# youtalk/opencv-ar

Hardware: AMD Instinct MI355X
Metric: frames/sec at 1920x1080, 16 markers/frame; 1/2/4/8 MI355X (higher is better)
Workload: dtype u8

## Files before the change

opencv-ar_amd/csrc/api.hip:

```cpp
#include "kernels.h"
#include "lanes_core.h"
#include <algorithm>
#include <cstdio>
#include <cstdlib>
#include <cstring>
#include <mutex>
#include <new>
#include <string>
#include <thread>
#include <vector>

using namespace ocvar;

static_assert(sizeof(TemplateRec) == sizeof(OcvarTemplate) && sizeof(TemplateRec) == 48, "CvarTemplate layout");
static_assert(MAX_SIZE_CLASSES == OCVAR_MAX_TEMPLATE_SIZES, "size classes");
static_assert(sizeof(CameraRec) == sizeof(OcvarCamera) && sizeof(CameraRec) == 248, "CvarCamera layout");
static_assert(sizeof(MarkerRec) == sizeof(OcvarMarker) && sizeof(MarkerRec) == 184, "CvarMarker layout");
static_assert(sizeof(BoardEntry) == sizeof(OcvarBoardMarker) && sizeof(BoardEntry) == 72, "OcvarBoardMarker layout");
static_assert(sizeof(BoardPose) == sizeof(OcvarBoardPose) && sizeof(BoardPose) == 192, "OcvarBoardPose layout");

struct OcvarGate {
    int device = 0;
    std::mutex mu;
    LaneSched sched;
// ... 1055 lines not shown
    for (int i = 0; i < n && i < max_quads; i++)
        for (int k = 0; k < 8; k++) quads[8 * i + k] = (int)sq[8 * (size_t)i + k];
    return OCVAR_OK;
}

extern "C" int ocvar_hip_debug_gray(OcvarHip* c, int frame, uint8_t* h) {
    if (!c || !h || frame < 0 || frame >= c->ws.n_frames) return OCVAR_E_ARG;
    HIP_TRY(c, hipSetDevice(c->device));
    const int W = c->ws.W, H = c->ws.H, pitch = gray_pitch(W);
    const size_t plane = (size_t)gray_plane_bytes(W, H);
    std::vector<uint8_t> g(plane);
    HIP_TRY(c, hipMemcpy(g.data(), c->ws.gray + frame * plane, plane, hipMemcpyDeviceToHost));
    for (int y = 0; y < H; y++)
        for (int x = 0; x < W; x++) h[(size_t)y * W + x] = g[(size_t)y * pitch + gray_col(x)];
    return OCVAR_OK;
}

extern "C" int ocvar_hip_debug_binary(OcvarHip* c, int frame, uint8_t* h) {
    if (!c || !h || frame < 0 || frame >= c->ws.n_frames) return OCVAR_E_ARG;
    HIP_TRY(c, hipSetDevice(c->device));
    const int sw = c->ws.sw, sh = c->ws.sh, ns = c->ws.ns;
    const size_t bytes = (size_t)nbr_plane_bytes(ns, sh);
    std::vector<uint8_t> nbr(bytes);
    HIP_TRY(c, hipMemcpy(nbr.data(), c->ws.nbr_frame + (size_t)frame * bytes, bytes, hipMemcpyDeviceToHost));
    for (int y = 0; y < sh; y++)
        for (int x = 0; x < sw; x++) h[(size_t)y * sw + x] = nbr_bit(nbr.data(), x, y, ns) ? 255 : 0;
    return OCVAR_OK;
}

extern "C" int ocvar_hip_debug_masks(OcvarHip* c, int frame, uint8_t* h) {
    if (!c || !h || frame < 0 || frame >= c->ws.n_frames) return OCVAR_E_ARG;
    HIP_TRY(c, hipSetDevice(c->device));
    const int sw = c->ws.sw, sh = c->ws.sh, ns = c->ws.ns;
    const size_t bytes = (size_t)nbr_plane_bytes(ns, sh);
    std::vector<uint8_t> nbr(bytes);
    HIP_TRY(c, hipMemcpy(nbr.data(), c->ws.nbr_frame + (size_t)frame * bytes, bytes, hipMemcpyDeviceToHost));
    for (int y = 0; y < sh; y++)
        for (int x = 0; x < sw; x++) h[(size_t)y * sw + x] = (uint8_t)nbr_of(nbr.data(), x, y, ns);
    return OCVAR_OK;
}

extern "C" int ocvar_hip_debug_frame_quads(OcvarHip* c, int frame, int* quads, int* n_quads) {
    if (!c || !quads || !n_quads || frame < 0 || frame >= c->ws.n_frames) return OCVAR_E_ARG;
    HIP_TRY(c, hipSetDevice(c->device));
    int n = 0;
    HIP_TRY(c, hipMemcpy(&n, c->ws.n_squares + frame, sizeof(int), hipMemcpyDeviceToHost));
    const int lim = c->ws.maxq < OCVAR_MAX_QUADS ? c->ws.maxq : OCVAR_MAX_QUADS;
    std::vector<float> sq((size_t)lim * 8);
    HIP_TRY(c, hipMemcpy(sq.data(), c->ws.squares + (size_t)frame * c->ws.maxq * 8, sq.size() * sizeof(float), hipMemcpyDeviceToHost));
    *n_quads = n;
    for (int i = 0; i < n && i < lim; i++)
        for (int k = 0; k < 8; k++) quads[8 * i + k] = (int)sq[8 * (size_t)i + k];
    return OCVAR_OK;
}

extern "C" int ocvar_hip_debug_candidates(OcvarHip* c, int frame, OcvarCandidate* cands, int max_cands, int* n_cands) {
    if (!c || !cands || !n_cands || frame < 0 || frame >= c->ws.n_frames) return OCVAR_E_ARG;
    HIP_TRY(c, hipSetDevice(c->device));
    int nsq = 0;
    HIP_TRY(c, hipMemcpy(&nsq, c->ws.n_squares + frame, sizeof(int), hipMemcpyDeviceToHost));
    if (nsq > c->ws.maxq) nsq = c->ws.maxq;
    const Workspace& w = c->ws;
    const Library& L = c->lib;
    const size_t first = (size_t)frame * w.maxq;
    std::vector<SquareRec> recs(nsq > 0 ? nsq : 1);
    std::vector<long long> codes((size_t)(nsq > 0 ? nsq : 1) * w.n_sizes);
    std::vector<int> match((size_t)(nsq > 0 ? nsq : 1) * w.max_match);
    if (nsq > 0) {
        HIP_TRY(c, hipMemcpy(recs.data(), w.sq_recs + first, nsq * sizeof(SquareRec), hipMemcpyDeviceToHost));
        HIP_TRY(c, hipMemcpy(codes.data(), w.sq_codes + first * w.n_sizes, codes.size() * sizeof(long long), hipMemcpyDeviceToHost));
        HIP_TRY(c, hipMemcpy(match.data(), w.sq_match + first * w.max_match, match.size() * sizeof(int), hipMemcpyDeviceToHost));
    }
    std::vector<int> orient_of(L.n_groups(), 0);
    long long n = 0;
    for (int i = 0; i < nsq; i++) {
        const SquareRec& r = recs[i];
        if (r.n_match < 0) continue;
        if (n >= max_cands) {
            n += w.n_templates;
            continue;
        }
        const int* m = match.data() + (size_t)i * w.max_match;
        for (int k = 0; k < r.n_match; k++) orient_of[match_group(m[k])] = match_orient_of(m[k]);
        int sh = 0;
        for (int j = 0; j < w.n_templates; j++, n++) {
            const int orient = orient_of[L.group_of[j]];
            sh = (sh + orient_shift(orient)) & 3;
            if (n >= max_cands) continue;
            OcvarCandidate& o = cands[n];
            o.markerId = i;
            o.templateId = j;
            o.orient = orient;
            o.valid = 1;
            o.bit = codes[(size_t)i * w.n_sizes + L.size_of[j]];
            shift_square(r.square, sh, o.square);
            std::memcpy(o.patPoint, r.patPoint, sizeof o.patPoint);
        }
        for (int k = 0; k < r.n_match; k++) orient_of[match_group(m[k])] = 0;
    }
    *n_cands = n > 0x7fffffff ? 0x7fffffff : (int)n;
    return OCVAR_OK;
}

extern "C" int ocvar_hip_stage_ms(OcvarHip* c, float* ms, int n) {
    if (!c || !ms || n < 1 || c->pending) return OCVAR_E_ARG;
    int k = 0;
    for (; k < 11 && k < n; k++)
        if (hipEventElapsedTime(&ms[k], c->ev[k], c->ev[k + 1]) != hipSuccess) ms[k] = -1.f;
    if (k < n && k == 11) {
        if (hipEventElapsedTime(&ms[11], c->ev[0], c->ev[12]) != hipSuccess) ms[11] = -1.f;
        k = 12;
    }
    return k;
}

extern "C" int ocvar_hip_stage_stamps(OcvarHip* c, void* ref_event, float* ms, int n) {
    if (!c || !ref_event || !ms || n < 1 || c->pending) return OCVAR_E_ARG;
    int k = 0;
    for (; k < 13 && k < n; k++)
        if (hipEventElapsedTime(&ms[k], (hipEvent_t)ref_event, c->ev[k]) != hipSuccess) {
            (void)hipGetLastError();
            ms[k] = -1.f;
        }
    return k;
}

__global__ void calib_copy_dword_kernel(const unsigned* src, unsigned* dst, size_t n) {
    for (size_t i = (size_t)blockIdx.x * blockDim.x + threadIdx.x; i < n; i += (size_t)gridDim.x * blockDim.x) dst[i] = src[i] + 1u;
}

extern "C" int ocvar_hip_debug_calibrate(OcvarHip* c, size_t bytes) {
    if (!c || bytes < 1024) return OCVAR_E_ARG;
    HIP_TRY(c, hipSetDevice(c->device));
    unsigned *a = nullptr, *b = nullptr;
    HIP_TRY(c, hipMalloc((void**)&a, bytes));
    HIP_TRY(c, hipMalloc((void**)&b, bytes));
    HIP_TRY(c, hipMemset(a, 1, bytes));
    hipLaunchKernelGGL(calib_copy_dword_kernel, dim3(4096), dim3(256), 0, c->stream, a, b, bytes / 4);
    HIP_TRY(c, hipStreamSynchronize(c->stream));
    (void)hipFree(a);
    (void)hipFree(b);
    return OCVAR_OK;
}

extern "C" int ocvar_hip_counters(OcvarHip* c, long long* out, int n) {
    if (!c || !out || n < 1 || c->pending) return OCVAR_E_ARG;
    const int* h = c->h_counters;
    long long v[10] = {h[CNT_FRAME_CANDS], h[CNT_CROP_ROIS], h[CNT_CROP_TILES], h[CNT_CROP_CANDS],
                      (long long)*reinterpret_cast<const unsigned long long*>(h + CNT_CROP_PIXELS),
                      (long long)*reinterpret_cast<const unsigned long long*>(h + CNT_POOL_INTS),
                      h[CNT_MID_F], h[CNT_MID_C], h[CNT_LONG_F], h[CNT_LONG_C]};
    int k = 0;
    for (; k < 10 && k < n; k++) out[k] = v[k];
    for (; k < 42 && k < n; k++) out[k] = (long long)reinterpret_cast<const unsigned long long*>(h + CNT_PROF)[k - 10];
    return k;
}
```

opencv-ar_amd/csrc/follow.hip:

```cpp
#include "kernels.h"
#include "trace_core.h"

namespace ocvar {

__device__ __forceinline__ int ticket_lane() {
    int l = (int)(threadIdx.x & 63);
    asm volatile("" : "+v"(l));
    return l;
}
__device__ __forceinline__ int uni(int v) { return __builtin_amdgcn_readfirstlane(v); }
__device__ __forceinline__ unsigned uni(unsigned v) { return (unsigned)__builtin_amdgcn_readfirstlane((int)v); }
__device__ __forceinline__ unsigned long long uni(unsigned long long v) {
    return ((unsigned long long)uni((unsigned)(v >> 32)) << 32) | uni((unsigned)v);
}
__device__ __forceinline__ double uni(double v) { return __longlong_as_double((long long)uni((unsigned long long)__double_as_longlong(v))); }

#ifdef OCVAR_PROF
#define PROF_NOW() __builtin_readcyclecounter()
#define PROF_DECL() unsigned long long prof_acc[16] = {0, 0, 0, 0, 0, 0, 0, 0, 0, 0, 0, 0, 0, 0, 0, 0}
#define PROF_ADD(slot, v) do { prof_acc[slot] += (unsigned long long)(v); } while (0)
#define PROF_FLUSH(base) do { if ((threadIdx.x & 63) == 0) for (int i_ = 0; i_ < 16; i_++) if (i_ != 7) atomicAdd(reinterpret_cast<unsigned long long*>(ws.counters + CNT_PROF) + (base) + i_, prof_acc[i_]); } while (0)
#else
#define PROF_NOW() 0ull
#define PROF_DECL() do { } while (0)
#define PROF_ADD(slot, v) do { (void)(v); } while (0)
#define PROF_FLUSH(base) do { } while (0)
#endif

constexpr int FW = 1;
constexpr int FOLLOW_THREADS = 64 * FW;

struct PlaneRef {
    const uint8_t* nbr;
    int ns, sh, img_w, img_h, plane;
};

template <bool CROP>
__device__ __forceinline__ PlaneRef plane_of(const Workspace& ws, int roi) {
    PlaneRef p;
    if (CROP) {
        const Roi r = ws.rois_crop[roi];
        p.ns = r.ns; p.sh = r.sh; p.img_w = r.w; p.img_h = r.h;
        p.nbr = ws.nbr_crop + r.nbr_off;
    } else {
        p.ns = ws.ns; p.sh = ws.sh; p.img_w = ws.W; p.img_h = ws.H;
        p.nbr = ws.nbr_frame + (size_t)roi * nbr_plane_bytes(ws.ns, ws.sh);
    }
    p.plane = p.ns * p.sh;
    return p;
}

template <bool CROP>
__device__ __forceinline__ void emit_quad(const Workspace& ws, const StartCand c, const int* dst);

template <bool CROP>
__device__ __forceinline__ void approximate_and_emit(const Workspace& ws, const StartCand c, const PlaneRef& pl, const int* pts,
                                                     int npts, double perimeter, DpSlice* stack, bool emit = true) {
    int dst[2 * (DP_MAX_OUT + 1)];
    const int m = approx_poly_dp(pts, npts, perimeter * 0.02, dst, stack);
    if (m != 4 || !quad_filter(dst, pl.img_w, pl.img_h)) return;
    if (emit) emit_quad<CROP>(ws, c, dst);
}

template <bool CROP>
__device__ __forceinline__ void emit_quad(const Workspace& ws, const StartCand c, const int* dst) {
    QuadRec q;
    q.roi = c.roi;
    q.start = c.pos;
    for (int k = 0; k < 8; k++) q.pt[k] = dst[k];
    if (CROP) {
        const int slot = atomicAdd(ws.counters + CNT_CROP_QUADS, 1);
        if (slot >= ws.cap_crop_quads) {
            atomicOr(ws.counters + CNT_ERR, ERR_QUAD_OVERFLOW);
            return;
        }
        ws.quads_crop[slot] = q;
        atomicMin(ws.best_crop + c.roi, ((unsigned long long)(unsigned)c.pos << 32) | (unsigned)slot);
    } else {
        const int slot = atomicAdd(ws.n_quads_frame + c.roi, 1);
        if (slot >= ws.maxq) {
            atomicOr(ws.counters + CNT_ERR, ERR_QUAD_OVERFLOW);
            return;
        }
        ws.quads_frame[(size_t)c.roi * ws.maxq + slot] = q;
    }
}

template <int CTRL, int ROWS = 0xf>
__device__ __forceinline__ unsigned dpp_self(unsigned v) {
    return (unsigned)__builtin_amdgcn_update_dpp((int)v, (int)v, CTRL, ROWS, 0xf, false);
}
template <int CTRL, int ROWS = 0xf>
__device__ __forceinline__ unsigned dpp_zero(unsigned v) {
    return (unsigned)__builtin_amdgcn_update_dpp(0, (int)v, CTRL, ROWS, 0xf, false);
}
#define OCVAR_WAVE_LADDER(STEP) \
    STEP(0xB1, 0xf) STEP(0x4E, 0xf) STEP(0x141, 0xf) STEP(0x140, 0xf) STEP(0x142, 0xa) STEP(0x143, 0xc)

__device__ __forceinline__ unsigned wave_max_u32(unsigned v) {
#define STEP(C, R) { const unsigned o = dpp_self<C, R>(v); v = o > v ? o : v; }
    OCVAR_WAVE_LADDER(STEP)
#undef STEP
    return (unsigned)__builtin_amdgcn_readlane((int)v, 63);
}
__device__ __forceinline__ unsigned long long wave_max_u64(unsigned long long v) {
#define STEP(C, R) { const unsigned long long o = ((unsigned long long)dpp_self<C, R>((unsigned)(v >> 32)) << 32) | dpp_self<C, R>((unsigned)v); v = o > v ? o : v; }
    OCVAR_WAVE_LADDER(STEP)
#undef STEP
    return ((unsigned long long)(unsigned)__builtin_amdgcn_readlane((int)(unsigned)(v >> 32), 63) << 32) |
           (unsigned)__builtin_amdgcn_readlane((int)(unsigned)v, 63);
}
typedef unsigned short us2v __attribute__((ext_vector_type(2)));
__device__ __forceinline__ unsigned pk_min(unsigned a, unsigned b) { return __builtin_bit_cast(unsigned, __builtin_elementwise_min(__builtin_bit_cast(us2v, a), __builtin_bit_cast(us2v, b))); }
__device__ __forceinline__ unsigned pk_max(unsigned a, unsigned b) { return __builtin_bit_cast(unsigned, __builtin_elementwise_max(__builtin_bit_cast(us2v, a), __builtin_bit_cast(us2v, b))); }
__device__ __forceinline__ unsigned wave_pk_min(unsigned v) {
#define STEP(C, R) v = pk_min(v, dpp_self<C, R>(v));
    OCVAR_WAVE_LADDER(STEP)
#undef STEP
    return (unsigned)__builtin_amdgcn_readlane((int)v, 63);
}
__device__ __forceinline__ unsigned wave_pk_max(unsigned v) {
#define STEP(C, R) v = pk_max(v, dpp_self<C, R>(v));
    OCVAR_WAVE_LADDER(STEP)
#undef STEP
    return (unsigned)__builtin_amdgcn_readlane((int)v, 63);
}
__device__ __forceinline__ double wave_sum_f64(double v) {
#define STEP(C, R) { const unsigned long long b = (unsigned long long)__double_as_longlong(v); \
                     v += __longlong_as_double((long long)(((unsigned long long)dpp_zero<C, R>((unsigned)(b >> 32)) << 32) | dpp_zero<C, R>((unsigned)b))); }
    OCVAR_WAVE_LADDER(STEP)
#undef STEP
    const unsigned long long b = (unsigned long long)__double_as_longlong(v);
    return __longlong_as_double((long long)(((unsigned long long)(unsigned)__builtin_amdgcn_readlane((int)(unsigned)(b >> 32), 63) << 32) |
                                            (unsigned)__builtin_amdgcn_readlane((int)(unsigned)b, 63)));
}

__device__ __forceinline__ int px_of(unsigned p) { return (int)(p & 0xffffu); }
__device__ __forceinline__ int py_of(unsigned p) { return (int)(p >> 16); }

constexpr int LDS_PTS = SLAB_PTS;
constexpr int DP_DST = 2 * (DP_MAX_OUT + 1);

struct WaveScratch {
    DpSlice stack[DP_STACK];
    int dst[DP_DST];
};

template <bool K32>
__device__ __forceinline__ int wave_approx_dp(const unsigned* src, int count, double parameter, int* dst, DpSlice* stack) {
    const int lane = threadIdx.x & 63;
    float eps = (float)parameter;
    eps *= eps;
    int top = 0, new_count = 0;
    DpSlice slice = {0, 0}, right = {0, 0};
    int sx = 0, sy = 0;
    bool le_eps = false;
    int pos = 0;
    for (int it = 0; it < 3; it++) {
        pos = (pos + right.start) % count;
        const unsigned sp = uni(src[pos]);
        sx = px_of(sp);
        sy = py_of(sp);
        int max_dist = 0;
        if (K32) {
            unsigned best = 0;
            for (int j = 1 + lane; j < count; j += 64) {
                int q = pos + j;
                q = q >= count ? q - count : q;
                const unsigned p = src[q];
                const int dx = px_of(p) - sx, dy = py_of(p) - sy;
                const unsigned dist = (unsigned)(dx * dx + dy * dy);
                const unsigned key = dist ? (dist << 11) | (~(unsigned)j & 0x7ffu) : 0u;
                best = key > best ? key : best;
            }
// ... 284 lines not shown
            }
            const int idx = tk_next + lane;
            tk_next += 64;
            bool alive = false;
            StartCand cc;
            cc.roi = 0; cc.pos = 0; cc.is_hole = 0;
            if (idx < tk_end) {
                cc = cands[idx];
                const PlaneRef pl = plane_of<CROP>(ws, cc.roi);
                const bool ring_done = !cc.is_hole && cc.pos == pl.ns + 1 && (CROP ? ws.ring_crop : ws.ring_frame)[cc.roi] != 0;
                if (!ring_done && cc.pos > 0 && cc.pos < pl.plane && !run_has_earlier_pixel_bits(pl.nbr, pl.ns, cc.pos, cc.is_hole))
                    alive = trace_flat(pl.nbr, pl.ns, pl.plane, cc.pos, cc.is_hole, nullptr, 0, PRE_STEPS).status == TRACE_OVERRUN;
            }
            const unsigned long long mask = __ballot(alive);
            if (alive) wqueue[wave][queued + __popcll(mask & below)] = cc;
            queued += __popcll(mask);
        }
        if (queued == 0) break;
        const int take = queued < 64 ? queued : 64;
        __builtin_amdgcn_fence(__ATOMIC_ACQ_REL, "workgroup");
        StartCand c;
        c.roi = 0; c.pos = 0; c.is_hole = 0;
        int route = 0;
        if (lane < take) {
            c = wqueue[wave][queued - take + lane];
            route = follow_short<CROP>(ws, c);
        }
        queued -= take;
        if (CROP && route == 1) atomicMin(ws.crop_min_rest + c.roi, c.pos);
        collect(0, o_n0, route == 1, c);
        collect(1, o_n1, route == 2, c);
        if (CROP) collect(2, o_n2, route == 3, c);
    }
    append(0, o_n0);
    append(1, o_n1);
    if (CROP) append(2, o_n2);
}

template <bool CROP>
__global__ __launch_bounds__(64) void ring_quads_kernel(Workspace ws) {
    int n = CROP ? ws.counters[CNT_CROP_ROIS] : ws.n_frames;
    if (CROP && n > ws.cap_crop_rois) n = ws.cap_crop_rois;
    int* ring = CROP ? ws.ring_crop : ws.ring_frame;
    const int lane = threadIdx.x;
    for (int roi = blockIdx.x; roi < n; roi += gridDim.x) {
        const PlaneRef pl = plane_of<CROP>(ws, roi);
        const int ns = uni(pl.ns), sh = uni(pl.sh), sw = uni(pl.img_w) & ~1;
        bool bad = sw < 8 || sh < 8;
        if (!bad) {
            const int tiles = ns >> 4;
            for (int i = lane; i < 2 * tiles; i += 64) {
                const int y = i < tiles ? 1 : sh - 2, xt = i < tiles ? i : i - tiles;
                const unsigned v = *reinterpret_cast<const unsigned*>(pl.nbr + nbr_win_off(xt << 4, y, ns) + 4);
                const int lo = (xt << 4) > 1 ? (xt << 4) : 1, hi = (xt << 4) + 15 < sw - 2 ? (xt << 4) + 15 : sw - 2;
                if (lo <= hi) {
                    const unsigned need = ((2u << (hi - lo)) - 1u) << (lo - (xt << 4) + 1);
                    if ((v & need) != need) bad = true;
                }
            }
            for (int y = 1 + lane; y <= sh - 2; y += 64)
                if (!nbr_bit(pl.nbr, 1, y, ns) || !nbr_bit(pl.nbr, sw - 2, y, ns)) bad = true;
        }
        const bool clean = __ballot(bad) == 0;
        if (lane == 0) {
            ring[roi] = clean ? 1 : 0;
            if (clean && (long long)(sw - 3) * (sh - 3) > 500) {
                const int pts[8] = {1, 1, 1, sh - 2, sw - 2, sh - 2, sw - 2, 1};
                const TraceStats st = stats_of_points(pts, 4);
                StartCand c;
                c.roi = roi;
                c.pos = ns + 1;
                c.is_hole = 0;
                DpSlice stack[DP_STACK];
                approximate_and_emit<CROP>(ws, c, pl, pts, 4, st.perimeter, stack);
            }
        }
    }
}

constexpr unsigned LW_EXIT = 0x1c00u;
constexpr unsigned LW_DELTA = 0x00030003u;

__device__ __forceinline__ unsigned lean_table_entry(unsigned idx) {
    const unsigned from = idx & 7u, t = idx >> 3;
    const unsigned e = (from + t) & 7u;
    const unsigned dx = (unsigned)(step_dx((int)e) + 1), dy = (unsigned)(step_dy((int)e) + 1);
    const unsigned pw = ((12u - from) & 7u) < t, pe = ((8u - from) & 7u) < t;
    return dx | (dy << 16) | (((e + 5u) & 7u) << 5) | (e << 10) | (pe << 30) | (pw << 31);
}

struct LeanWalk {
    unsigned xy;
    unsigned m;
    unsigned from;
    unsigned pe;
    unsigned xy0, xy1;
    unsigned cxy;
    int npts, step, status;
};

__device__ __forceinline__ void lean_begin(LeanWalk& w, const uint8_t* nbr, int ns, int cpos, int is_hole) {
    const int i0 = cpos - is_hole;
    const int x = i0 % ns, y = i0 / ns;
    w.xy = w.xy0 = (unsigned)x | ((unsigned)y << 16);
    w.cxy = w.xy0 + (unsigned)is_hole;
    w.npts = 0;
    w.step = 0;
    w.status = -1;
    w.xy1 = 0;
    w.pe = 0;
    w.from = 0;
    w.m = nbr_of(nbr, x, y, ns);
    if (w.m == 0) {
        w.status = TRACE_SINGLE;
        w.npts = 1;
        return;
    }
    const int s = first_cw(w.m, (is_hole ? 0 : 4) - 1);
    w.xy1 = w.xy0 + (unsigned)(step_dx(s) + 65536 * step_dy(s));
    w.pe = (unsigned)(s ^ 4) << 10;
    w.from = (unsigned)(s + 1) & 7u;
}

template <class Park>
__device__ __forceinline__ void lean_step(LeanWalk& w, const unsigned* tab, const uint8_t* base, unsigned nt, unsigned last, Park&& park) {
    const unsigned mm = __builtin_amdgcn_perm(w.m, w.m, 0u);
    const unsigned t = (unsigned)__builtin_ctz(__builtin_amdgcn_alignbit(mm, mm, w.from));
    const unsigned ent = tab[(t << 3) + w.from];
    const int d = (int)(w.xy - w.cxy);
    const unsigned nf = ((ent << 1) & (unsigned)(d + 1)) | (ent & (unsigned)d);
    const unsigned nxy = w.xy + (ent & LW_DELTA) - 0x10001u;
    const bool closes = (nxy == w.xy0) & (w.xy == w.xy1);
    const unsigned e = ent & LW_EXIT;
    const bool emit = e != w.pe;
    unsigned off = nbr_win_off_xy(nxy, nt);
    off = off < last ? off : last;
    const unsigned* win = reinterpret_cast<const unsigned*>(base + off);
    const unsigned m4 = nbr_mask9(win[0], win[1], win[2], nxy & 15u);
    park(w.xy);
    w.npts += emit ? 1 : 0;
    w.status = (int)nf < 0 ? (int)TRACE_NOT_FIRST : closes ? (int)TRACE_OK : m4 == 0u ? (int)TRACE_OVERRUN : -1;
    w.step += 1;
    w.xy = nxy;
    w.pe = e;
    w.from = (ent >> 5) & 7u;
    w.m = m4;
}

constexpr int MID_BLOCK = 32;
constexpr int POINT_ROW = MID_BLOCK + 1;
constexpr int FLUSH_W = MID_BLOCK <= 16 ? 16 : 32;
static_assert(FLUSH_W >= MID_BLOCK && 64 % FLUSH_W == 0, "a group of lanes covers a whole row of parked points");

template <bool CROP>
__global__ __launch_bounds__(FOLLOW_THREADS) void follow_mid_kernel(Workspace ws, int phase) {
    __shared__ WaveScratch scratch[FW];
    __shared__ unsigned parked[FW][64 * POINT_ROW];
    __shared__ unsigned step_tab[64];
    if (threadIdx.x < 64u) step_tab[threadIdx.x] = lean_table_entry(threadIdx.x);
    __syncthreads();
    const StartCand* cands = CROP ? ws.mid_crop : ws.mid_frame;
    StartCand* longs = CROP ? ws.long_crop : ws.long_frame;
    int n = ws.counters[CROP ? CNT_MID_C : CNT_MID_F];
    if (n > ws.cap_long) n = ws.cap_long;
    int n_first = (CROP && phase != 2) ? ws.counters[CNT_MID_C_FIRST] : 0;
    if (n_first > ws.cap_long) n_first = ws.cap_long;
    n += n_first;
    int* ticket = ws.counters + (CROP ? (phase == 2 ? CNT_TICKET_MC2 : CNT_TICKET_MC) : CNT_TICKET_MF);
    int* n_long = ws.counters + (CROP ? CNT_LONG_C : CNT_LONG_F);
    const int lane = threadIdx.x & 63;
    const int wave = uni((int)(threadIdx.x >> 6));
    const unsigned long long below = (1ull << lane) - 1ull;
    unsigned* wave_slabs = reinterpret_cast<unsigned*>(ws.slab) + ((size_t)blockIdx.x * blockDim.x + uni((int)(threadIdx.x & ~63u))) * SLAB_STRIDE;
    static_assert(64 * POINT_ROW >= LDS_PTS, "the staging area of the approximation aliases the (flushed) point rows");
    unsigned* my_row = parked[wave] + lane * POINT_ROW;
    const unsigned* wave_rows = parked[wave];
    int flushed = 0;
    const int budget = ws.mid_steps;
    bool have = false;
    bool more = true;
    StartCand c;
    c.roi = 0; c.pos = 0; c.is_hole = 0;
    PlaneRef pl = plane_of<CROP>(ws, 0);
    LeanWalk w;
    w.xy = w.m = w.from = w.pe = w.xy0 = w.xy1 = w.cxy = 0u;
    w.npts = w.step = 0;
    w.status = TRACE_NOT_FIRST;
    unsigned pl_nt = 1u, pl_last = 0u;
    long long guard = ((long long)n + 64) * (budget / MID_BLOCK + 5) + 64;
    PROF_DECL();
    for (;;) {
        if (--guard < 0) {
            if (lane == 0) atomicOr(ws.counters + CNT_ERR, ERR_TICKET_RUNAWAY);
            break;
        }
        const unsigned long long pt0 = PROF_NOW();
        for (int tries = 0; tries < (CROP ? 4 : 1); tries++) {
            const unsigned long long idle = __ballot(!have);
            if (!(more && idle)) break;
            if (tries > 0) --guard;
            const int cnt = __popcll(idle);
            int base = 0;
            if (ticket_lane() == 0) base = atomicAdd(ticket, cnt);
            base = uni(base);
            if (base + cnt >= n) more = false;
            if (!have) {
                const int idx = base + __popcll(idle & below);
                if (idx < n) {
                    c = (CROP && idx < n_first) ? ws.mid_first_crop[idx] : cands[idx - n_first];
                    bool take = true;
                    if (CROP) {
                        const int earliest = ws.crop_min_rest[c.roi];
                        const bool beaten = (unsigned)(ws.best_crop[c.roi] >> 32) < (unsigned)c.pos;
                        if (phase == 1) take = idx < n_first || c.pos == earliest;
                        else if (phase == 2) take = c.pos != earliest && !beaten;
                        else take = !beaten;
                    }
                    pl = plane_of<CROP>(ws, c.roi);
                    if (take && c.pos > 0 && c.pos < pl.plane) {
                        lean_begin(w, pl.nbr, pl.ns, c.pos, c.is_hole);
                        pl_nt = (unsigned)(pl.ns >> 4);
                        pl_last = (unsigned)nbr_plane_bytes(pl.ns, pl.sh) - 12u;
                        have = true;
                        flushed = 0;
                    }
                }
            }
        }
        if (__ballot(have) == 0) break;
        const unsigned long long pt1 = PROF_NOW();
        PROF_ADD(0, pt1 - pt0);
        for (int k = 0; k < MID_BLOCK; k++) {
            const bool running = have && w.status < 0;
            if (__ballot(running) == 0) break;
            PROF_ADD(4, 1);
            PROF_ADD(5, __popcll(__ballot(running)));
            if (running)
                lean_step(w, step_tab, pl.nbr, pl_nt, pl_last, [&](unsigned xy) {
                    const int slot = w.npts - flushed;
                    my_row[slot < MID_BLOCK ? slot : MID_BLOCK] = xy;
                });
        }
        if (have && w.status < 0 && w.step >= budget) w.status = TRACE_OVERRUN;
        const unsigned long long pt2 = PROF_NOW();
        PROF_ADD(1, pt2 - pt1);
        {
            const int stored = w.npts < SLAB_PTS ? w.npts : SLAB_PTS;
            const int pend = have ? stored - flushed : 0;
            unsigned long long fm = __ballot(pend > 0);
            if (fm) __builtin_amdgcn_fence(__ATOMIC_ACQ_REL, "workgroup");
            const int grp = lane / FLUSH_W, k = lane % FLUSH_W;
            while (fm) {
                int L = 0, cnt = 0, off = 0;
#pragma unroll
                for (int g = 0; g < 64 / FLUSH_W; g++) {
                    const int Lg = fm ? __ffsll((long long)fm) - 1 : 0;
                    const int cg = fm ? __builtin_amdgcn_readlane(pend, Lg) : 0;
                    const int og = __builtin_amdgcn_readlane(flushed, Lg);
                    fm &= fm - 1;
                    L = grp == g ? Lg : L;
                    cnt = grp == g ? cg : cnt;
                    off = grp == g ? og : off;
                }
                if (k < cnt) wave_slabs[(size_t)L * SLAB_STRIDE + off + k] = wave_rows[L * POINT_ROW + k];
            }
            flushed += pend;
        }
        const unsigned long long pt3 = PROF_NOW();
        PROF_ADD(2, pt3 - pt2);
        int route = 0, slab_npts = 0;
#ifdef OCVAR_PROF
        {
            const bool done = have && w.status >= 0;
            for (int st_ = 0; st_ < 3; st_++) {
                const int want = st_ == 0 ? (int)TRACE_NOT_FIRST : st_ == 1 ? (int)TRACE_OK : (int)TRACE_OVERRUN;
                const bool mine = done && w.status == want;
                PROF_ADD(9 + 2 * st_, __popcll(__ballot(mine)));
                unsigned steps_ = mine ? (unsigned)w.step : 0u;
                for (int o_ = 32; o_ > 0; o_ >>= 1) steps_ += (unsigned)__shfl_xor((int)steps_, o_, 64);
                PROF_ADD(8 + 2 * st_, steps_);
            }
            bool useless = false;
            if (CROP && done && w.status == TRACE_OK) useless = (unsigned)(ws.best_crop[c.roi] >> 32) < (unsigned)c.pos;
            unsigned us_ = useless ? (unsigned)w.step : 0u;
            for (int o_ = 32; o_ > 0; o_ >>= 1) us_ += (unsigned)__shfl_xor((int)us_, o_, 64);
            PROF_ADD(14, us_);
            PROF_ADD(15, __popcll(__ballot(done && w.status == TRACE_OK && w.npts < 4)));
        }
#endif
        if (have && w.status >= 0) {
            if (w.status == TRACE_OVERRUN) route = 1;
            else if (w.status == TRACE_OK && w.npts >= 4) {
                if (w.npts <= SLAB_PTS) {
                    route = 3;
                    slab_npts = w.npts;
                } else {
                    route = follow_overflow<CROP>(ws, c, pl);
                }
            }
            have = false;
        }
        unsigned long long todo = __ballot(route == 3);
        unsigned my_best = 0xffffffffu;
        if (CROP && route == 3) my_best = (unsigned)(ws.best_crop[c.roi] >> 32);
        if (todo) __builtin_amdgcn_fence(__ATOMIC_ACQ_REL, "workgroup");
        while (todo) {
            const int L = __ffsll((long long)todo) - 1;
            todo &= todo - 1;
            StartCand cl;
            cl.roi = __builtin_amdgcn_readlane(c.roi, L);
            cl.pos = __builtin_amdgcn_readlane(c.pos, L);
            cl.is_hole = __builtin_amdgcn_readlane(c.is_hole, L);
            const int nl = __builtin_amdgcn_readlane(slab_npts, L);
            const unsigned* sl = wave_slabs + (size_t)L * SLAB_STRIDE;
            PlaneRef pll = pl;
            pll.img_w = __builtin_amdgcn_readlane(pl.img_w, L);
            pll.img_h = __builtin_amdgcn_readlane(pl.img_h, L);
            const bool beaten = CROP && (unsigned)__builtin_amdgcn_readlane((int)my_best, L) < (unsigned)cl.pos;
            if (!beaten) wave_finish_packed<CROP, true>(ws, cl, pll, sl, nl, parked[wave], &scratch[wave]);
            PROF_ADD(6, 1);
        }
        PROF_ADD(3, PROF_NOW() - pt3);
        const unsigned long long mask = __ballot(route == 1);
        if (mask) {
            int qbase = 0;
            const int leader = __ffsll((long long)mask) - 1;
            if (lane == leader) qbase = atomicAdd(n_long, __popcll(mask));
            qbase = __builtin_amdgcn_readlane(qbase, leader);
            if (route == 1) {
                const int slot = qbase + __popcll(mask & below);
                if (slot < ws.cap_long) longs[slot] = c;
                else atomicOr(ws.counters + CNT_ERR, ERR_CAND_OVERFLOW);
            }
        }
    }
    PROF_FLUSH(CROP ? 16 : 0);
}

constexpr int TILE_SLOTS = TILE_H + 2;
struct TileCache {
    unsigned* lds;
    const uint8_t* nbr;
    int ns, sh;
    int tx0, ty0;
};

__device__ __forceinline__ void tile_load(TileCache& t, int x, int y, int bx = 0, int by = 0) {
    const int lane = threadIdx.x & 63;
    t.tx0 = (x + 20 * bx - TILE_W / 2 + 8) & ~15;
    t.ty0 = (int)div14((unsigned)(y + 24 * by - 28 + 4 * NBR_TILE_H)) * NBR_TILE_H - 4 * NBR_TILE_H;
    const int tx = (t.tx0 >> 4), ty = t.ty0 / NBR_TILE_H, nty = (t.sh + NBR_TILE_H - 1) / NBR_TILE_H;
    constexpr int NQ = TILE_TX * TILE_TY * 4;
    static_assert(NQ > 64 && NQ <= 128, "two quarter tiles per lane at most");
    uint4 v[2];
#pragma unroll
    for (int h = 0; h < 2; h++) {
        const int q = lane + 64 * h, i = (q >> 2) % TILE_TX, j = (q >> 2) / TILE_TX;
        v[h] = make_uint4(0u, 0u, 0u, 0u);
        if (q < NQ && tx + i >= 0 && (tx + i) * 16 < t.ns && ty + j >= 0 && ty + j < nty)
            v[h] = *reinterpret_cast<const uint4*>(t.nbr + nbr_tile_off((unsigned)(tx + i), (unsigned)(ty + j), t.ns) + 16 * (q & 3));
    }
#pragma unroll
    for (int h = 0; h < 2; h++) {
        const int q = lane + 64 * h, i = (q >> 2) % TILE_TX, j = (q >> 2) / TILE_TX;
        if (q < NQ) {
            unsigned* d = t.lds + i * TILE_SLOTS + NBR_TILE_H * j + 4 * (q & 3);
            d[0] = v[h].x; d[1] = v[h].y; d[2] = v[h].z; d[3] = v[h].w;
        }
    }
    __builtin_amdgcn_fence(__ATOMIC_ACQ_REL, "workgroup");
}

__device__ __forceinline__ unsigned tile_mask(const TileCache& t, int lx, int ly) {
    const unsigned* w = t.lds + ((unsigned)lx >> 4) * TILE_SLOTS + (unsigned)ly;
    return nbr_mask9(w[0], w[1], w[2], (unsigned)lx & 15u);
}

__device__ __forceinline__ unsigned tile_get(TileCache& t, int x, int y) {
    if ((unsigned)(x - t.tx0) >= (unsigned)TILE_W || (unsigned)(y - t.ty0) >= (unsigned)TILE_H) tile_load(t, x, y);
    return uni(tile_mask(t, x - t.tx0, y - t.ty0));
}

__device__ LeanTrace trace_lean_tiled(TileCache& t, int cpos, int is_hole, int* out, int max_pts, int max_steps) {
    const int lane = threadIdx.x & 63;
    LeanTrace r;
    r.status = TRACE_OK;
    r.npts = 0;
    r.steps = 0;
    const int ns = t.ns;
    const int i0 = cpos - is_hole;
    const int x0 = i0 % ns, y0 = i0 / ns;
    int x = x0, y = y0;
    unsigned m = tile_get(t, x, y);
    if (m == 0) {
        r.status = TRACE_SINGLE;
        r.npts = 1;
        return r;
    }
    int s = first_cw(m, (is_hole ? 0 : 4) - 1);
    const int x1 = x0 + step_dx(s), y1 = y0 + step_dy(s);
    int prev_s = s ^ 4;
    int straight = 0;
    int step = 0;
    unsigned hp = 0;
    unsigned* out1 = reinterpret_cast<unsigned*>(out);
    for (;; step++) {
        if (step >= max_steps) {
            r.status = TRACE_OVERRUN;
            break;
        }
        const int from = (s + 1) & 7;
        const int tz = __builtin_ctz(((m * 0x101u) >> from) & 0xffu);
        const int e = (from + tz) & 7;
        const unsigned passed = ((((1u << tz) - 1u) * 0x101u) << from) >> 8;
        const int idx = y * ns + x;
        if (((passed & 0x10u) && idx < cpos) || ((passed & 1u) && idx + 1 < cpos)) {
            r.status = TRACE_NOT_FIRST;
            break;
        }
        if (e != prev_s) {
            if (r.npts < max_pts) {
                const int slot = r.npts & 63;
                hp = lane == slot ? ((unsigned)x | ((unsigned)y << 16)) : hp;
                if (slot == 63) out1[r.npts - 63 + lane] = hp;
            }
            r.npts++;
            prev_s = e;
        }
        const int ddx = step_dx(e), ddy = step_dy(e);
        const int px = x, py = y;
        x += ddx;
        y += ddy;
        if (x == x0 && y == y0 && px == x1 && py == y1) break;
        if ((unsigned)x >= (unsigned)ns || (unsigned)y >= (unsigned)t.sh) {
            r.status = TRACE_OVERRUN;
            break;
        }
        unsigned m4 = tile_get(t, x, y);
        if (m4 == 0) {
            r.status = TRACE_OVERRUN;
            break;
        }
        if (e == (s ^ 4) && m4 == m) {
            if (++straight >= 2) {
                bool closed = false, bad = false;
                for (;;) {
                    const int qx = x + (lane + 1) * ddx, qy = y + (lane + 1) * ddy;
                    const bool in_tile = (unsigned)(qx - t.tx0) < (unsigned)TILE_W && (unsigned)(qy - t.ty0) < (unsigned)TILE_H;
                    const unsigned mq = in_tile ? tile_mask(t, qx - t.tx0, qy - t.ty0) : 256u;
                    const bool closes = qx == x0 && qy == y0 && qx - ddx == x1 && qy - ddy == y1;
                    const unsigned long long close_mask = __ballot(closes);
                    const unsigned long long stop = close_mask | __ballot(mq != m);
                    const int k = stop ? __ffsll((long long)stop) - 1 : 64;
                    const int pa = y * ns + x, pb = (y + k * ddy) * ns + x + k * ddx;
                    if (((passed & 0x10u) && (pa < cpos || pb < cpos)) || ((passed & 1u) && (pa + 1 < cpos || pb + 1 < cpos))) {
                        r.status = TRACE_NOT_FIRST;
                        bad = true;
                        break;
                    }
                    x += k * ddx;
                    y += k * ddy;
                    step += k;
                    if (step >= max_steps) {
                        r.status = TRACE_OVERRUN;
                        bad = true;
                        break;
                    }
                    if (k == 64) continue;
                    if ((close_mask >> k) & 1ull) {
                        closed = true;
                        break;
                    }
                    const unsigned stop_m = (unsigned)__builtin_amdgcn_readlane((int)mq, k);
// ... 357 lines not shown
```

opencv-ar_amd/csrc/kernels.h:

```cpp
#pragma once
#include "hd.h"
#include "decode_core.h"
#include "pose_core.h"
#include "tail_core.h"
#include "refine_core.h"
#include "board_core.h"
#include "ocvar_hip.h"

namespace ocvar {

constexpr int MAXQ_DEFAULT = OCVAR_MAX_QUADS;
constexpr int MAXM = OCVAR_MAX_MARKERS;
constexpr int MAXT = OCVAR_MAX_TEMPLATES;
constexpr int MARCH_HALO_L = 2, MARCH_HALO_R = 2;
constexpr int MARCH_STRIP = 4 * (64 - MARCH_HALO_L - MARCH_HALO_R);
static_assert(MARCH_STRIP == GRAY_PANEL_COLS && 4 * MARCH_HALO_L == GRAY_PANEL_LEAD && 4 * 64 == GRAY_PANEL_BYTES, "a grey panel is what one wave of the frame kernel converts");
constexpr int MARCH_CROP_ROWS = 252;
constexpr int MARCH_STAGE = 512;
constexpr int BACK_STEPS = 32;
constexpr int PRE_STEPS = 8;
constexpr int SHORT_STEPS = 96;
constexpr int MID_STEPS = 1536;
constexpr int SLAB_PTS = 1024;
constexpr int SLAB_STRIDE = SLAB_PTS + 4;
constexpr int MID_BLOCKS_MAX = 1024;
constexpr int SLAB3_PTS = 8192;
constexpr int SLAB3_STRIDE = SLAB3_PTS + 64;
constexpr int LONG_BLOCKS_MAX = 1024;
constexpr int TILE_TX = 4, TILE_TY = 5;
constexpr int TILE_W = TILE_TX * NBR_TILE_W, TILE_H = TILE_TY * NBR_TILE_H;

enum { ERR_CAND_OVERFLOW = 1, ERR_POOL_OVERFLOW = 2, ERR_QUAD_OVERFLOW = 4, ERR_TRACE_OVERRUN = 8, ERR_CROP_OVERFLOW = 16,
       ERR_TILE_OVERFLOW = 32,
       ERR_TICKET_RUNAWAY = 64,
       ERR_MARKER_OVERFLOW = 128 };

struct TileDesc { int roi, x0, y0; };

struct SquareRec {
    float square[8];
    float patPoint[8];
    int n_match;
    int pad;
};

enum { CNT_FRAME_CANDS = 0, CNT_CROP_ROIS = 1, CNT_CROP_TILES = 2, CNT_CROP_CANDS = 3,
       CNT_POOL_INTS = 4 , CNT_CROP_QUADS = 6, CNT_TICKET_F = 7, CNT_TICKET_C = 8, CNT_ERR = 9,
       CNT_CROP_PIXELS = 10 , CNT_LONG_F = 12, CNT_LONG_C = 13, CNT_TICKET_LF = 14, CNT_TICKET_LC = 15,
       CNT_MID_F = 16, CNT_MID_C = 17, CNT_TICKET_MF = 18, CNT_TICKET_MC = 19, CNT_TICKET_BC = 20, CNT_MID_C_FIRST = 21, CNT_TICKET_MC2 = 22,
       CNT_POSE_JOBS = 23,
       CNT_PROF = 24 , CNT_COUNT = 88 };

struct Workspace {
    int max_w, max_h, max_batch;
    int maxq;
    int maxm;
    int dense;
    int track_gw, track_gh;
    int decode_slices;
    int order_chunk;
    int cap_frame_cands, cap_crop_cands, cap_crop_rois, cap_crop_tiles, cap_crop_quads;
    long long cap_pool_ints, cap_crop_pixels;
    int W, H, sw, sh, ns, n_frames, n_templates;
    int n_sizes, n_groups, max_match;
    int crop_phases;
    int mid_steps, mid_blocks, long_blocks;
    int max_mid_blocks, max_long_blocks;
    int short_blocks, crop_blocks;
    int frame_strips, frame_chunks, frame_chunk_rows;
    uint8_t* gray;
    uint8_t* nbr_frame;
    uint8_t* nbr_crop;
    StartCand* cands_frame;
    StartCand* cands_crop;
    StartCand* mid_frame;
    StartCand* mid_crop;
    StartCand* mid_first_crop;
    StartCand* long_frame;
    StartCand* long_crop;
    int cap_long;
    int* pool;
    int* slab;
    int* slab3;
    QuadRec* quads_frame;
    int* n_quads_frame;
    float* squares;
    int* n_squares;
    int* crop_of;
    Roi* rois_crop;
    TileDesc* tiles_crop;
    unsigned long long* crop_pixels;
    QuadRec* quads_crop;
    unsigned long long* best_crop;
    int* ring_frame;
    int* ring_crop;
    int* crop_min_rest;
    SquareRec* sq_recs;
    long long* sq_codes;
    int* sq_match;
    MarkerRec* prev;
    int* n_prev;
    int* reserve;
    int* n_reserve;
    int* pose_jobs;
    MarkerRec* markers;
    int* sorted_starts;
    float* sq_tmp;
    int* trk_cells;
    int* trk_fill;
    int* trk_items;
    int* trk_next;
    int* surv;
    int* src;
    int* n_markers;
    TemplateRec* templates;
    SizeClass* sizes;
    LutEntry* lut;
    int* group_off;
    int* group_members;
    CameraRec* camera;
    int* counters;
};

int input_format_bpp(int format);

void launch_binarise_frames(const Workspace& ws, const uint8_t* d_bgr, int row_stride, size_t frame_stride, int grey_in_place,
                            int format, hipStream_t stream);
void launch_binarise_crops(const Workspace& ws, hipStream_t stream);
void launch_ring_quads_frames(const Workspace& ws, hipStream_t stream);
void launch_ring_quads_crops(const Workspace& ws, hipStream_t stream);
void launch_follow_frames(const Workspace& ws, hipStream_t stream);
void launch_follow_crops(const Workspace& ws, hipStream_t stream);
void launch_follow_mid_frames(const Workspace& ws, hipStream_t stream);
void launch_follow_mid_crops(const Workspace& ws, hipStream_t stream);
void launch_follow_long_frames(const Workspace& ws, hipStream_t stream);
void launch_follow_long_crops(const Workspace& ws, hipStream_t stream);
void launch_order_and_crops(const Workspace& ws, hipStream_t stream);
void launch_decode(const Workspace& ws, hipStream_t stream);
void launch_finalise(const Workspace& ws, const RefineArgs& refine, hipStream_t stream);
void launch_refine_corners(const Workspace& ws, const RefineArgs& refine, hipStream_t stream);

struct BoardArgs {
    int n;
    const BoardEntry* entries;
    const int* map;
    BoardPose* poses;
};
void launch_board_poses(const Workspace& ws, const BoardArgs& board, hipStream_t stream);

}
```

Baseline: 249,700.

## Batch finished mid-kernel contours and finish four at once per wave quarter

In the mid follow kernel, traced contours whose points fit in the slab are no longer finished one at a time by the whole wave right away. Lanes now park them as waiting until at least FINISH_WAIT are ready, or no more work remains. Up to four contours of at most 512 points are then finished together, each by a 16-lane quarter doing its own bounding box, perimeter and Douglas-Peucker approximation with DPP row reductions. Larger or wide-coordinate contours still fall back to the whole-wave finish. This aims to raise lane use in the finishing step, but a waiting lane holds its slot and takes no new tickets, and each quarter needs its own scratch in shared memory.

After: 245,700. 1.6% lower.

```diff
diff --git a/opencv-ar_amd/csrc/api.hip b/opencv-ar_amd/csrc/api.hip
--- a/opencv-ar_amd/csrc/api.hip
+++ b/opencv-ar_amd/csrc/api.hip
@@ -1231,6 +1231,6 @@
                       h[CNT_MID_F], h[CNT_MID_C], h[CNT_LONG_F], h[CNT_LONG_C]};
     int k = 0;
     for (; k < 10 && k < n; k++) out[k] = v[k];
-    for (; k < 42 && k < n; k++) out[k] = (long long)reinterpret_cast<const unsigned long long*>(h + CNT_PROF)[k - 10];
+    for (; k < 46 && k < n; k++) out[k] = (long long)reinterpret_cast<const unsigned long long*>(h + CNT_PROF)[k - 10];
     return k;
 }
diff --git a/opencv-ar_amd/csrc/follow.hip b/opencv-ar_amd/csrc/follow.hip
--- a/opencv-ar_amd/csrc/follow.hip
+++ b/opencv-ar_amd/csrc/follow.hip
@@ -17,9 +17,10 @@
 
 #ifdef OCVAR_PROF
 #define PROF_NOW() __builtin_readcyclecounter()
-#define PROF_DECL() unsigned long long prof_acc[16] = {0, 0, 0, 0, 0, 0, 0, 0, 0, 0, 0, 0, 0, 0, 0, 0}
+#define PROF_DECL() unsigned long long prof_acc[18] = {0, 0, 0, 0, 0, 0, 0, 0, 0, 0, 0, 0, 0, 0, 0, 0, 0, 0}
 #define PROF_ADD(slot, v) do { prof_acc[slot] += (unsigned long long)(v); } while (0)
-#define PROF_FLUSH(base) do { if ((threadIdx.x & 63) == 0) for (int i_ = 0; i_ < 16; i_++) if (i_ != 7) atomicAdd(reinterpret_cast<unsigned long long*>(ws.counters + CNT_PROF) + (base) + i_, prof_acc[i_]); } while (0)
+#define PROF_FLUSH(base) do { if ((threadIdx.x & 63) == 0) for (int i_ = 0; i_ < 16; i_++) if (i_ != 7) atomicAdd(reinterpret_cast<unsigned long long*>(ws.counters + CNT_PROF) + (base) + i_, prof_acc[i_]); \
+    if ((threadIdx.x & 63) == 0) for (int i_ = 0; i_ < 2; i_++) atomicAdd(reinterpret_cast<unsigned long long*>(ws.counters + CNT_PROF) + 32 + (base) / 8 + i_, prof_acc[16 + i_]); } while (0)
 #else
 #define PROF_NOW() 0ull
 #define PROF_DECL() do { } while (0)
@@ -610,10 +611,269 @@
 constexpr int FLUSH_W = MID_BLOCK <= 16 ? 16 : 32;
 static_assert(FLUSH_W >= MID_BLOCK && 64 % FLUSH_W == 0, "a group of lanes covers a whole row of parked points");
 
+constexpr int Q_PTS = 512;
+constexpr int Q_ROW = 16 * POINT_ROW;
+static_assert(Q_ROW >= Q_PTS && Q_ROW % 4 == 0 && Q_PTS % 256 == 0, "a quarter's staging area holds Q_PTS points, 16-byte aligned");
+static_assert(Q_PTS <= 1024, "32-bit keys of the maximum searches");
+
+#define OCVAR_ROW_LADDER(STEP) STEP(0xB1) STEP(0x4E) STEP(0x141) STEP(0x140)
+__device__ __forceinline__ unsigned row_max_u32(unsigned v) {
+#define STEP(C) { const unsigned o = dpp_self<C>(v); v = o > v ? o : v; }
+    OCVAR_ROW_LADDER(STEP)
+#undef STEP
+    return v;
+}
+__device__ __forceinline__ unsigned row_pk_min(unsigned v) {
+#define STEP(C) v = pk_min(v, dpp_self<C>(v));
+    OCVAR_ROW_LADDER(STEP)
+#undef STEP
+    return v;
+}
+__device__ __forceinline__ unsigned row_pk_max(unsigned v) {
+#define STEP(C) v = pk_max(v, dpp_self<C>(v));
+    OCVAR_ROW_LADDER(STEP)
+#undef STEP
+    return v;
+}
+__device__ __forceinline__ double row_sum_f64(double v) {
+#define STEP(C) { const unsigned long long b = (unsigned long long)__double_as_longlong(v); \
+                  v += __longlong_as_double((long long)(((unsigned long long)dpp_self<C>((unsigned)(b >> 32)) << 32) | dpp_self<C>((unsigned)b))); }
+    OCVAR_ROW_LADDER(STEP)
+#undef STEP
+    return v;
+}
+
+__device__ __forceinline__ int quarter_approx_dp(const unsigned* src, int count, bool act, double parameter, int* dst, DpSlice* stack) {
+    const int gl = threadIdx.x & 15;
+    const int cnt = act ? count : 0;
+    float eps = (float)parameter;
+    eps *= eps;
+    int top = 0, new_count = 0, result = act ? -1 : 0;
+    int s_start = 0, s_end = 0, r_start = 0, r_end = 0;
+    int sx = 0, sy = 0;
+    bool le_eps = false;
+    int pos = 0;
+    for (int it = 0; it < 3; it++) {
+        pos += r_start;
+        pos -= pos >= cnt ? cnt : 0;
+        const unsigned sp = src[pos];
+        sx = px_of(sp);
+        sy = py_of(sp);
+        unsigned best = 0;
+        for (int j0 = 1 + gl; j0 < cnt; j0 += 64) {
+#pragma unroll
+            for (int u = 0; u < 4; u++) {
+                const int j = j0 + 16 * u;
+                const bool valid = j < cnt;
+                int q = pos + j;
+                q = q >= cnt ? q - cnt : q;
+                const unsigned p = src[valid ? q : 0];
+                const int dx = px_of(p) - sx, dy = py_of(p) - sy;
+                const unsigned dist = (unsigned)(dx * dx + dy * dy);
+                const unsigned key = (valid && dist) ? (dist << 11) | (~(unsigned)j & 0x7ffu) : 0u;
+                best = key > best ? key : best;
+            }
+        }
+        best = row_max_u32(best);
+        const int max_dist = (int)(best >> 11);
+        if (best) r_start = (int)(~best & 0x7ffu);
+        le_eps = (float)max_dist <= eps;
+    }
+    if (act) {
+        if (le_eps) {
+            dst[0] = sx;
+            dst[1] = sy;
+            new_count = 1;
+        } else {
+            s_start = pos;
+            s_end = r_start += s_start;
+            r_start -= r_start >= cnt ? cnt : 0;
+            r_end = s_start;
+            if (r_end < r_start) r_end += cnt;
+            stack[0].start = r_start; stack[0].end = r_end;
+            stack[1].start = s_start; stack[1].end = s_end;
+            top = 2;
+        }
+    }
+    int guard = 4 * cnt + 16;
+    while (__ballot(top > 0)) {
+        bool on = top > 0;
+        if (on && --guard < 0) {
+            result = DP_MAX_OUT + 1;
+            top = 0;
+            on = false;
+        }
+        const int t = on ? top - 1 : 0;
+        s_start = on ? stack[t].start : 0;
+        s_end = on ? stack[t].end : 0;
+        const int e = s_end >= cnt ? s_end - cnt : s_end;
+        const int b = s_start >= cnt ? s_start - cnt : s_start;
+        const unsigned ep = src[e], bp = src[b];
+        const int ex = px_of(ep), ey = py_of(ep);
+        sx = px_of(bp);
+        sy = py_of(bp);
+        const int dx = ex - sx, dy = ey - sy;
+        const bool wide = s_end > s_start + 1;
+        const int hi = wide ? s_end : 0;
+        unsigned best = 0;
+        for (int i0 = s_start + 1 + gl; i0 < hi; i0 += 64) {
+#pragma unroll
+            for (int u = 0; u < 4; u++) {
+                const int i = i0 + 16 * u;
+                const bool valid = i < hi;
+                const int q = i >= cnt ? i - cnt : i;
+                const unsigned p = src[valid ? q : 0];
+                int d = (py_of(p) - sy) * dx - (px_of(p) - sx) * dy;
+                d = d < 0 ? -d : d;
+                const unsigned key = (valid && d) ? ((unsigned)d << 11) | (~(unsigned)i & 0x7ffu) : 0u;
+                best = key > best ? key : best;
+            }
+        }
+        best = row_max_u32(best);
+        const int max_dist = (int)(best >> 11);
+        if (best) r_start = (int)(~best & 0x7ffu);
+        le_eps = !wide || (double)max_dist * max_dist <= (double)eps * ((double)dx * dx + (double)dy * dy);
+        if (on) {
+            if (le_eps) {
+                if (new_count >= DP_MAX_OUT) {
+                    result = DP_MAX_OUT + 1;
+                    top = 0;
+                } else {
+                    dst[2 * new_count] = sx;
+                    dst[2 * new_count + 1] = sy;
+                    new_count++;
+                    top = t;
+                }
+            } else {
+                r_end = s_end;
+                s_end = r_start;
+                if (new_count + t + 2 > DP_MAX_OUT) {
+                    result = DP_MAX_OUT + 1;
+                    top = 0;
+                } else {
+                    stack[t].start = r_start; stack[t].end = r_end;
+                    stack[t + 1].start = s_start; stack[t + 1].end = s_end;
+                    top = t + 2;
+                }
+            }
+        }
+    }
+    if (result < 0) {
+        const int n = new_count;
+        int r = n - 1;
+        sx = dst[2 * r];
+        sy = dst[2 * r + 1];
+        if (++r >= n) r = 0;
+        int wpos = r;
+        int px = dst[2 * r], py = dst[2 * r + 1];
+        if (++r >= n) r = 0;
+        for (int i = 0; i < n && new_count > 2; i++) {
+            const int ex = dst[2 * r], ey = dst[2 * r + 1];
+            if (++r >= n) r = 0;
+            const int dx = ex - sx, dy = ey - sy;
+            int dist = (px - sx) * dy - (py - sy) * dx;
+            dist = dist < 0 ? -dist : dist;
+            if ((double)dist * dist <= 0.5 * eps * (dx * dx + dy * dy) && dx != 0 && dy != 0) {
+                new_count--;
+                dst[2 * wpos] = sx = ex;
+                dst[2 * wpos + 1] = sy = ey;
+                if (++wpos >= n) wpos = 0;
+                px = dst[2 * r];
+                py = dst[2 * r + 1];
+                if (++r >= n) r = 0;
+                i++;
+                continue;
+            }
+            dst[2 * wpos] = sx = px;
+            dst[2 * wpos + 1] = sy = py;
+            if (++wpos >= n) wpos = 0;
+            px = ex;
+            py = ey;
+        }
+        result = new_count;
+    }
+    return result;
+}
+
+template <bool CROP>
+__device__ __forceinline__ bool quarter_finish(const Workspace& ws, bool on, int roi, int pos, int img_w, int img_h, const unsigned* gsrc, int npts,
+                                               unsigned* lq, WaveScratch* sc) {
+    const int gl = threadIdx.x & 15;
+    const int n = on ? npts : 0;
+    unsigned lo = 0xffffffffu, hi = 0u;
+    for (int k0 = 0; __ballot(k0 < n); k0 += 256) {
+        uint4 v[4];
+#pragma unroll
+        for (int k = 0; k < 4; k++) {
+            const int i = k0 + 4 * (gl + 16 * k);
+            v[k] = make_uint4(0u, 0u, 0u, 0u);
+            if (i < n) v[k] = *reinterpret_cast<const uint4*>(gsrc + i);
+        }
+#pragma unroll
+        for (int k = 0; k < 4; k++) {
+            const int i = k0 + 4 * (gl + 16 * k);
+            if (i < n) {
+                *reinterpret_cast<uint4*>(lq + i) = v[k];
+                const unsigned e[4] = {v[k].x, v[k].y, v[k].z, v[k].w};
+#pragma unroll
+                for (int c = 0; c < 4; c++) {
+                    const bool valid = i + c < n;
+                    lo = pk_min(lo, valid ? e[c] : 0xffffffffu);
+                    hi = pk_max(hi, valid ? e[c] : 0u);
+                }
+            }
+        }
+    }
+    lo = row_pk_min(lo);
+    hi = row_pk_max(hi);
+    const int bw = px_of(hi) - px_of(lo), bh = py_of(hi) - py_of(lo);
+    bool act = n >= 4 && (long long)bw * bh > 500;
+    const bool wide_keys = act && !((long long)bw * bw + (long long)bh * bh < (1ll << 21));
+    act = act && !wide_keys;
+    __builtin_amdgcn_fence(__ATOMIC_ACQ_REL, "workgroup");
+    const int np = act ? n : 0;
+    double per = 0.0;
+    for (int i0 = gl; i0 < np; i0 += 64) {
+#pragma unroll
+        for (int u = 0; u < 4; u++) {
+            const int i = i0 + 16 * u;
+            const bool valid = i < np;
+            const int ic = valid ? i : 0;
+            const unsigned p = lq[ic], q = lq[ic == 0 ? np - 1 : ic - 1];
+            const float dx = (float)px_of(p) - (float)px_of(q), dy = (float)py_of(p) - (float)py_of(q);
+            per += valid ? (double)sqrt_rn(dx * dx + dy * dy) : 0.0;
+        }
+    }
+    per = row_sum_f64(per);
+#ifdef OCVAR_PROF
+    if (act && gl == 0) atomicAdd(reinterpret_cast<unsigned long long*>(ws.counters + CNT_PROF) + (CROP ? 16 : 0) + 7, 1ull);
+#endif
+    const int m = quarter_approx_dp(lq, n, act, per * 0.02, sc->dst, sc->stack);
+    if (m == 4) {
+        int q[8];
+#pragma unroll
+        for (int k = 0; k < 8; k++) q[k] = sc->dst[k];
+        if (quad_filter(q, img_w, img_h) && gl == 0) {
+            StartCand c;
+            c.roi = roi;
+            c.pos = pos;
+            c.is_hole = 0;
+            emit_quad<CROP>(ws, c, q);
+        }
+    }
+    return wide_keys;
+}
+
+#ifndef OCVAR_FINISH_WAIT
+#define OCVAR_FINISH_WAIT 4
+#endif
+constexpr int FINISH_WAIT = OCVAR_FINISH_WAIT;
+static_assert(FINISH_WAIT >= 1 && FINISH_WAIT <= 64, "borders a wave waits for before it finishes them");
+
 template <bool CROP>
 __global__ __launch_bounds__(FOLLOW_THREADS) void follow_mid_kernel(Workspace ws, int phase) {
-    __shared__ WaveScratch scratch[FW];
-    __shared__ unsigned parked[FW][64 * POINT_ROW];
+    __shared__ WaveScratch scratch[FW][4];
+    __shared__ __attribute__((aligned(16))) unsigned parked[FW][64 * POINT_ROW];
     __shared__ unsigned step_tab[64];
     if (threadIdx.x < 64u) step_tab[threadIdx.x] = lean_table_entry(threadIdx.x);
     __syncthreads();
@@ -636,6 +896,8 @@
     int flushed = 0;
     const int budget = ws.mid_steps;
     bool have = false;
+    bool waiting = false;
+    int slab_npts = 0;
     bool more = true;
     StartCand c;
     c.roi = 0; c.pos = 0; c.is_hole = 0;
@@ -654,7 +916,7 @@
         }
         const unsigned long long pt0 = PROF_NOW();
         for (int tries = 0; tries < (CROP ? 4 : 1); tries++) {
-            const unsigned long long idle = __ballot(!have);
+            const unsigned long long idle = __ballot(!have && !waiting);
             if (!(more && idle)) break;
             if (tries > 0) --guard;
             const int cnt = __popcll(idle);
@@ -662,7 +924,7 @@
             if (ticket_lane() == 0) base = atomicAdd(ticket, cnt);
             base = uni(base);
             if (base + cnt >= n) more = false;
-            if (!have) {
+            if (!have && !waiting) {
                 const int idx = base + __popcll(idle & below);
                 if (idx < n) {
                     c = (CROP && idx < n_first) ? ws.mid_first_crop[idx] : cands[idx - n_first];
@@ -685,7 +947,7 @@
                 }
             }
         }
-        if (__ballot(have) == 0) break;
+        if (__ballot(have || waiting) == 0) break;
         const unsigned long long pt1 = PROF_NOW();
         PROF_ADD(0, pt1 - pt0);
         for (int k = 0; k < MID_BLOCK; k++) {
@@ -726,7 +988,7 @@
         }
         const unsigned long long pt3 = PROF_NOW();
         PROF_ADD(2, pt3 - pt2);
-        int route = 0, slab_npts = 0;
+        int route = 0;
 #ifdef OCVAR_PROF
         {
             const bool done = have && w.status >= 0;
@@ -752,31 +1014,59 @@
                 if (w.npts <= SLAB_PTS) {
                     route = 3;
                     slab_npts = w.npts;
+                    waiting = true;
                 } else {
                     route = follow_overflow<CROP>(ws, c, pl);
                 }
             }
             have = false;
         }
-        unsigned long long todo = __ballot(route == 3);
-        unsigned my_best = 0xffffffffu;
-        if (CROP && route == 3) my_best = (unsigned)(ws.best_crop[c.roi] >> 32);
-        if (todo) __builtin_amdgcn_fence(__ATOMIC_ACQ_REL, "workgroup");
-        while (todo) {
-            const int L = __ffsll((long long)todo) - 1;
-            todo &= todo - 1;
-            StartCand cl;
-            cl.roi = __builtin_amdgcn_readlane(c.roi, L);
-            cl.pos = __builtin_amdgcn_readlane(c.pos, L);
-            cl.is_hole = __builtin_amdgcn_readlane(c.is_hole, L);
-            const int nl = __builtin_amdgcn_readlane(slab_npts, L);
-            const unsigned* sl = wave_slabs + (size_t)L * SLAB_STRIDE;
-            PlaneRef pll = pl;
-            pll.img_w = __builtin_amdgcn_readlane(pl.img_w, L);
-            pll.img_h = __builtin_amdgcn_readlane(pl.img_h, L);
-            const bool beaten = CROP && (unsigned)__builtin_amdgcn_readlane((int)my_best, L) < (unsigned)cl.pos;
-            if (!beaten) wave_finish_packed<CROP, true>(ws, cl, pll, sl, nl, parked[wave], &scratch[wave]);
-            PROF_ADD(6, 1);
+        const unsigned long long wm = __ballot(waiting);
+        if (wm && (__popcll(wm) >= FINISH_WAIT || !more || __ballot(have) == 0)) {
+            unsigned my_best = 0xffffffffu;
+            if (CROP && waiting) my_best = (unsigned)(ws.best_crop[c.roi] >> 32);
+            const bool live = waiting && !(CROP && my_best < (unsigned)c.pos);
+            unsigned long long qm = __ballot(live && slab_npts <= Q_PTS);
+            unsigned long long whole = __ballot(live && slab_npts > Q_PTS);
+            __builtin_amdgcn_fence(__ATOMIC_ACQ_REL, "workgroup");
+            PROF_ADD(6, __popcll(wm));
+            const int grp = lane >> 4;
+            while (qm) {
+                PROF_ADD(16, 1);
+                PROF_ADD(17, __popcll(qm) < 4 ? __popcll(qm) : 4);
+                int myL = 0;
+                bool on = false;
+#pragma unroll
+                for (int g = 0; g < 4; g++) {
+                    const bool has = qm != 0;
+                    const int Lg = has ? __ffsll((long long)qm) - 1 : 0;
+                    qm &= qm - 1;
+                    myL = grp == g ? Lg : myL;
+                    on = grp == g ? has : on;
+                }
+                const int q_roi = __shfl(c.roi, myL, 64), q_pos = __shfl(c.pos, myL, 64), q_n = __shfl(slab_npts, myL, 64);
+                const int q_w = __shfl(pl.img_w, myL, 64), q_h = __shfl(pl.img_h, myL, 64);
+                const bool wide = quarter_finish<CROP>(ws, on, q_roi, q_pos, q_w, q_h, wave_slabs + (size_t)myL * SLAB_STRIDE, q_n,
+                                                       parked[wave] + grp * Q_ROW, &scratch[wave][grp]);
+#pragma unroll
+                for (int g = 0; g < 4; g++)
+                    if (__builtin_amdgcn_readlane((int)wide, 16 * g)) whole |= 1ull << __builtin_amdgcn_readlane(myL, 16 * g);
+            }
+            while (whole) {
+                const int L = __ffsll((long long)whole) - 1;
+                whole &= whole - 1;
+                StartCand cl;
+                cl.roi = __builtin_amdgcn_readlane(c.roi, L);
+                cl.pos = __builtin_amdgcn_readlane(c.pos, L);
+                cl.is_hole = __builtin_amdgcn_readlane(c.is_hole, L);
+                const int nl = __builtin_amdgcn_readlane(slab_npts, L);
+                const unsigned* sl = wave_slabs + (size_t)L * SLAB_STRIDE;
+                PlaneRef pll = pl;
+                pll.img_w = __builtin_amdgcn_readlane(pl.img_w, L);
+                pll.img_h = __builtin_amdgcn_readlane(pl.img_h, L);
+                wave_finish_packed<CROP, true>(ws, cl, pll, sl, nl, parked[wave], &scratch[wave][0]);
+            }
+            waiting = false;
         }
         PROF_ADD(3, PROF_NOW() - pt3);
         const unsigned long long mask = __ballot(route == 1);
diff --git a/opencv-ar_amd/csrc/kernels.h b/opencv-ar_amd/csrc/kernels.h
--- a/opencv-ar_amd/csrc/kernels.h
+++ b/opencv-ar_amd/csrc/kernels.h
@@ -49,7 +49,7 @@
        CNT_CROP_PIXELS = 10 , CNT_LONG_F = 12, CNT_LONG_C = 13, CNT_TICKET_LF = 14, CNT_TICKET_LC = 15,
        CNT_MID_F = 16, CNT_MID_C = 17, CNT_TICKET_MF = 18, CNT_TICKET_MC = 19, CNT_TICKET_BC = 20, CNT_MID_C_FIRST = 21, CNT_TICKET_MC2 = 22,
        CNT_POSE_JOBS = 23,
-       CNT_PROF = 24 , CNT_COUNT = 88 };
+       CNT_PROF = 24 , CNT_COUNT = 96 };
 
 struct Workspace {
     int max_w, max_h, max_batch;
```
